# martinhoT/Footsies-Gym

Hardware: NVIDIA B200
Metric: env_frames_per_sec (higher is better)
Workload: dtype int32+fp32

## Files before the change

### footsies_gym_b200/csrc/frame_logic.cuh

```cuda
#ifndef FOOTSIES_B200_FRAME_LOGIC_CUH
#define FOOTSIES_B200_FRAME_LOGIC_CUH

#include <stdint.h>

#include "state_codec.h"

#if defined(__CUDACC__)
#define FG_DEV __device__ __forceinline__
#define FG_ALIGN16 __align__(16)
namespace fg {
FG_DEV float u2f(uint32_t u) { return __uint_as_float(u); }
FG_DEV uint32_t f2u(float f) { return __float_as_uint(f); }
FG_DEV uint32_t umulhi64(uint32_t r, unsigned long long m) { return (uint32_t)__umul64hi((unsigned long long)r, m); }
FG_DEV uint32_t byte_lut(uint32_t lo, uint32_t hi, uint32_t idx) { return __byte_perm(lo, hi, idx); }
FG_DEV uint32_t umin(uint32_t a, uint32_t b) { return min(a, b); }
}
#else
#include <math.h>
#include <string.h>
#define FG_DEV static inline
#define FG_ALIGN16 alignas(16)
struct uint2 { uint32_t x, y; };
struct FG_ALIGN16 uint4 { uint32_t x, y, z, w; };
namespace fg {
FG_DEV float u2f(uint32_t u) { float f; memcpy(&f, &u, 4); return f; }
FG_DEV uint32_t f2u(float f) { uint32_t u; memcpy(&u, &f, 4); return u; }
FG_DEV uint32_t umulhi64(uint32_t r, unsigned long long m) { return (uint32_t)(((unsigned __int128)r * m) >> 64); }
FG_DEV uint32_t byte_lut(uint32_t lo, uint32_t hi, uint32_t idx) {
    const unsigned long long t = (unsigned long long)hi << 32 | lo;
    uint32_t r = 0;
    for (int k = 0; k < 4; k++) r |= (uint32_t)((t >> (8 * ((idx >> (4 * k)) & 7u))) & 0xffu) << (8 * k);
    return r;
}
FG_DEV uint32_t umin(uint32_t a, uint32_t b) { return a < b ? a : b; }
}
#endif

namespace fg {

enum : uint32_t { STAND = FT_IDX_STAND, FORWARD = FT_IDX_FORWARD, BACKWARD = FT_IDX_BACKWARD,
                  DASH_FORWARD = FT_IDX_DASH_FORWARD, DASH_BACKWARD = FT_IDX_DASH_BACKWARD,
                  N_ATTACK = FT_IDX_N_ATTACK, B_ATTACK = FT_IDX_B_ATTACK, N_SPECIAL = FT_IDX_N_SPECIAL,
                  B_SPECIAL = FT_IDX_B_SPECIAL, DAMAGE = FT_IDX_DAMAGE, GUARD_BREAK = FT_IDX_GUARD_BREAK,
                  GUARD_PROXIMITY = FT_IDX_GUARD_PROXIMITY, DEAD = FT_IDX_DEAD, WIN = FT_IDX_WIN };

constexpr int kMovePatBytes = 408;
constexpr int kAttPatBytes = 256;

struct BoxCfg { uint32_t h0cx, h0hw, h1cx, h1hw, pcx, pw, r0, r1; };
struct AttackRow { uint32_t pcx, phw, rcx, rhw, pybits, rybits, result, r0; };
struct BotRow { unsigned long long magic_m, magic_a; uint32_t n_m, sel_m, n_a, sel_a; };

struct FG_ALIGN16 Tables {
    uint4 rows[FT_NUM_ROWS];
    BoxCfg boxcfg[16];
    AttackRow attack[8];
    BotRow bot[8];
    double term_reward[FT_NUM_CUM][4][2];
    double step_reward[4];
    uint8_t cum_next[16][4];
    uint32_t move_meta[8], att_meta[8];
    uint8_t bucket_of[16];
    uint16_t dash_fsm[256][4];
    uint8_t arun_lut[64 * 8];
    uint8_t req_lut[2][1024];
    uint8_t move_pat[2][kMovePatBytes];
    uint8_t att_pat[kAttPatBytes];
};
static_assert(sizeof(Tables) % 16 == 0, "Tables is copied as uint4");
static_assert(sizeof(BoxCfg) == 32 && sizeof(AttackRow) == 32 && sizeof(BotRow) == 32, "byte offsets are pre-positioned");

struct StatAcc { uint32_t a, r, s, ep_frames; };
constexpr uint32_t kStatFlushFrames = 120u;

struct Env {
    float pos1, vel1, pos2, vel2;
    uint32_t pk1, hist1, pk2, hist2;
    int32_t frame;
    uint32_t misc, bq2, bq1;
    uint32_t r0, r1, r2, r3;
    bool drew;
};

constexpr uint32_t M_FRAME1 = 1u << FGP_FRAME_SHIFT, M_ACT = 31u << FGP_ACT_SHIFT, M_STUN = 31u << FGP_STUN_SHIFT,
                   M_STUN1 = 1u << FGP_STUN_SHIFT, M_GUARD = 3u << FGP_GUARD_SHIFT, M_GUARD1 = 1u << FGP_GUARD_SHIFT,
                   M_VITAL = 1u << FGP_VITAL_SHIFT, M_HIT = 1u << FGP_HITCNT_SHIFT, M_BUF = 1u << FGP_BUF_SHIFT,
                   M_RSV = 1u << FGP_RSV_SHIFT, M_INBACK = 1u << FGP_INBACK_SHIFT, M_RPROX = 1u << FGP_RPROX_SHIFT,
                   M_SHMAG = 7u << FGP_SHAKE_SHIFT, M_SHMAG1 = 1u << FGP_SHAKE_SHIFT, M_SHSIGN = 1u << FGP_SHAKE_SIGN_SHIFT;

FG_DEV uint32_t rng_next(Env &e) {
    uint32_t t = e.r0 ^ (e.r0 << 11);
    e.r0 = e.r1; e.r1 = e.r2; e.r2 = e.r3;
    e.r3 = e.r3 ^ (e.r3 >> 19) ^ t ^ (t >> 8);
    e.drew = true;
    return e.r3;
}

struct FrameOut {
    uint32_t z, w;
    float pos_b;
    bool special_started;
    bool from_neutral;
};

template <int SIDE, bool LUT_REQUEST>
FG_DEV void update_fighter(const Tables &T, uint32_t in, float &pos, float &vel, uint32_t &pk, uint32_t &hist, FrameOut &fo) {
    const uint32_t in_lr = in & 3u;
    const uint32_t au = T.arun_lut[((hist >> (FGH_ARUN_SHIFT - 3)) & (63u << 3)) + in];
    const uint32_t du = T.dash_fsm[hist & 255u][in_lr];
    hist = (du & 255u) | (au & 63u) << FGH_ARUN_SHIFT;
    uint32_t delta = (pk & M_STUN) ? (0u - M_STUN1) : M_FRAME1;
    if (pk & M_SHMAG) { delta -= M_SHMAG1; pk ^= M_SHSIGN; }
    pk += delta;
    const bool stun0 = (pk & M_STUN) == 0u;

    uint32_t req;
    bool differs, set, want_buffer;
    if (LUT_REQUEST) {
        static_assert(FGP_RPROX_SHIFT == 23 && FGP_CARRY_END == (1u << 28), "request LUT index assembly");
        const uint32_t ridx = in_lr | ((pk >> 21) & 0x384u) | ((au >> 3) & 0x18u) | ((du >> 3) & 0x60u);
        const uint32_t rq = T.req_lut[SIDE][ridx];
        req = rq & 15u;
        differs = ((pk ^ (req << FGP_ACT_SHIFT)) & M_ACT) != 0u;
        set = (rq & FT_REQ_FREE) && ((rq & FT_REQ_ENDED) || differs);
        want_buffer = (rq & FT_REQ_WANT_BUFFER) != 0u;
    } else {
        const bool special = (au & 64u) != 0u;
        const bool atk_down = (au & 128u) != 0u;
        const bool dash_f = (du & (SIDE == 0 ? 0x200u : 0x100u)) != 0u;
        const bool dash_b = (du & (SIDE == 0 ? 0x100u : 0x200u)) != 0u;
        const bool ended = (pk & FGP_CARRY_END) != 0u;
        const bool in_normal = (pk & FGP_CARRY_NORMAL) && !ended;
        const uint32_t dir = in_lr != 0u ? 1u : 0u;
        const uint32_t areq = special ? N_SPECIAL + dir : in_normal ? (uint32_t)N_SPECIAL : N_ATTACK + dir;
        const uint32_t mv = byte_lut(SIDE == 0 ? 0x00010200u : 0x00020100u, SIDE == 0 ? 0x00010e00u : 0x000e0100u,
                                     in_lr | ((pk >> (FGP_RPROX_SHIFT - 2)) & 4u));
        req = (special || atk_down) ? areq : dash_f ? (uint32_t)DASH_FORWARD : dash_b ? (uint32_t)DASH_BACKWARD : mv;
        const bool free_to_switch = ended || (pk & FGP_CARRY_ALWAYS);
        differs = ((pk ^ (req << FGP_ACT_SHIFT)) & M_ACT) != 0u;
        set = free_to_switch && (ended || differs);
        want_buffer = !free_to_switch && req == N_SPECIAL;
    }
    const bool normal = (pk & FGP_CARRY_NORMAL) != 0u;
    if ((pk & (M_RSV | M_BUF)) && stun0 && ((pk & M_RSV) || (pk & M_HIT))) {
        req = (pk & M_RSV) ? (uint32_t)GUARD_BREAK : (uint32_t)N_SPECIAL;
        set = true; differs = true; want_buffer = false;
    } else {
        pk = (pk & ~(M_INBACK | M_RPROX)) | (in & (SIDE == 0 ? 1u : 2u)) << (FGP_INBACK_SHIFT - (SIDE == 0 ? 0 : 1));
    }
    if (SIDE == 0) {
        fo.special_started = set && differs && (req - N_SPECIAL) < 2u;
        fo.from_neutral = !normal;
    }
    if (set) pk = (pk & (M_STUN | M_GUARD | M_VITAL | M_INBACK | M_RPROX)) + (req << FGP_ACT_SHIFT);

    const uint4 row = T.rows[pk & FGP_ROW_MASK];
    if (want_buffer) pk |= (row.z & FT_Z_CANCEL) << (FGP_BUF_SHIFT - 3);
    pk = (pk & ~FGP_CARRY_MASK) | (row.w & (stun0 ? FGP_CARRY_MASK : (FGP_CARRY_MASK & ~FGP_CARRY_END)));

    if (stun0) {
        const float dx = u2f(row.x);
        pos = pos + (SIDE == 0 ? dx : -dx);
        if (row.z & FT_Z_HAS_MOVEMENT) vel = u2f(row.y);
    }
    fo.z = row.z;
    fo.w = row.w;
    fo.pos_b = pos;
}

FG_DEV const BoxCfg &boxcfg_of(const Tables &T, uint32_t z) {
    return *reinterpret_cast<const BoxCfg *>(reinterpret_cast<const char *>(T.boxcfg) + (z & (15u << FT_Z_BOXCFG_SHIFT)));
}
FG_DEV const AttackRow &attack_of(const Tables &T, uint32_t w) {
    return *reinterpret_cast<const AttackRow *>(reinterpret_cast<const char *>(T.attack) + (w & (7u << FT_W_KIND_SHIFT)));
}
static_assert(FT_Z_BOXCFG_SHIFT == 5 && FT_W_KIND_SHIFT == 5, "id << 5 == byte offset of a 32-byte table row");
static_assert(FT_Z_CANCEL == 8u, "update_fighter shifts the cancel bit into the buffered-cancel bit");

template <int SIDE>
FG_DEV void box_extent(float pos_b, uint32_t cx_bits, uint32_t hw_bits, float s, float t, float &lo, float &hi) {
    const float cx = u2f(cx_bits), hw = u2f(hw_bits);
    const float x = ((pos_b + (SIDE == 0 ? cx : -cx)) + s) + t;
    lo = x - hw;
    hi = x + hw;
}

template <int ASIDE>
FG_DEV void attack_overlaps(const AttackRow &ar, const BoxCfg &vb, const FrameOut &af, const FrameOut &vf, float a_s,
                            float a_t, float v_s, float v_t, bool &real_hit, bool &prox_hit) {
    float plo, phi, rlo, rhi, v0lo, v0hi, v1lo, v1hi;
    box_extent<ASIDE>(af.pos_b, ar.pcx, ar.phw, a_s, a_t, plo, phi);
    box_extent<ASIDE>(af.pos_b, ar.rcx, ar.rhw, a_s, a_t, rlo, rhi);
    box_extent<1 - ASIDE>(vf.pos_b, vb.h0cx, vb.h0hw, v_s, v_t, v0lo, v0hi);
    box_extent<1 - ASIDE>(vf.pos_b, vb.h1cx, vb.h1hw, v_s, v_t, v1lo, v1hi);
    constexpr uint32_t Y0 = 0xffu << FT_Z_YMASK0_SHIFT, Y1 = 0xffu << FT_Z_YMASK1_SHIFT;
    const bool r0 = (vf.z & ar.rybits & Y0) && v0hi >= rlo && v0lo <= rhi;
    const bool r1 = (vf.z & ar.rybits & Y1) && v1hi >= rlo && v1lo <= rhi;
    const bool p0 = (vf.z & ar.pybits & Y0) && v0hi >= plo && v0lo <= phi;
    const bool p1 = (vf.z & ar.pybits & Y1) && v1hi >= plo && v1lo <= phi;
    real_hit = (af.z & FT_Z_REAL) && (r0 || r1);
    prox_hit = (af.z & FT_Z_PROX) && (p0 || p1);
}

template <int ASIDE>
FG_DEV uint32_t attack_apply(uint32_t result, uint32_t &apk, uint32_t &vpk, const FrameOut &af, const FrameOut &vf,
                             bool real_hit, bool prox_hit, StatAcc &acc) {
    const bool can = (af.z & (FT_Z_PROX | FT_Z_REAL)) && !(apk & M_HIT);
    if (can && real_hit) {
        const bool brk = (vpk & M_GUARD) == 0u;
        const bool guarding = (vf.z & FT_Z_GUARDING) != 0u;
        uint32_t nact, stun, res;
        uint32_t keep = vpk & (M_GUARD | M_VITAL | M_INBACK | M_RPROX);
        if (!brk) keep -= M_GUARD1;
        if (guarding) {
            nact = (result >> 5) & 31u;
            stun = brk ? (result >> 21) & 31u : (result >> 16) & 31u;
            if (brk) keep |= M_RSV;
            res = brk ? 3u : 6u;
            acc.r += brk ? (1u << 24) : (1u << 16);
        } else {
            if (result & (1u << 10)) keep &= ~M_VITAL;
            nact = result & 31u;
            stun = (result >> 11) & 31u;
            res = brk ? 1u : 5u;
            acc.r += 1u << 8;
        }
        const uint32_t mag = umin(stun / 3u, 6u);
        vpk = keep | nact << FGP_ACT_SHIFT | stun << FGP_STUN_SHIFT | mag << FGP_SHAKE_SHIFT
            | (ASIDE == 0 ? 0u : (mag ? M_SHSIGN : 0u));
        apk = (apk & ~(M_STUN | (stun ? FGP_CARRY_END : 0u))) | stun << FGP_STUN_SHIFT | M_HIT;
        return res;
    }
    if (can && prox_hit) vpk |= (vpk & M_INBACK) << (FGP_RPROX_SHIFT - FGP_INBACK_SHIFT);
    return 0u;
}

FG_DEV uint32_t bot_dist_index(float dist) {
    float t2 = dist * 2.0f;
    t2 = t2 < 4.0f ? 4.0f : t2 > 9.0f ? 9.0f : t2;
    return (uint32_t)((int)ceilf(t2) - 4);
}
FG_DEV float bot_dist_of_index(uint32_t idx) { return 0.5f * (float)(idx + 4u); }

template <int SIDE>
FG_DEV uint32_t bot_next(const Tables &T, Env &e, uint32_t &q, float dist, uint32_t opp_act) {
    uint32_t input = 0u;
    const bool have_m = (q & (127u << 9)) != 0u, have_a = (q & (127u << 24)) != 0u;
    if (have_m) {
        input = T.move_pat[SIDE][q & 511u];
        q += 1u - (1u << 9);
    }
    if (have_a) {
        input |= T.att_pat[(q >> 16) & 255u];
        q += (1u << 16) - (1u << 24);
    }
    if (!(have_m && have_a)) {
        const BotRow &b = T.bot[T.bucket_of[bot_dist_index(dist)]];
        if (!have_m) {
            const uint32_t r = rng_next(e);
            const uint32_t k = r - umulhi64(r, b.magic_m) * b.n_m;
            const uint32_t meta = T.move_meta[(b.sel_m >> (4u * k)) & 15u];
            q = (q & 0xffff0000u) | (meta & 0xffffu) | (meta >> 16) << 9;
        }
        if (!have_a) {
            const bool opp_hurt = opp_act == DAMAGE || opp_act == GUARD_BREAK || opp_act == N_SPECIAL || opp_act == B_SPECIAL;
            const bool opp_normal = opp_act == N_ATTACK || opp_act == B_ATTACK;
            uint32_t ap = 3u;
            if (!(opp_hurt || (opp_normal && (b.n_a >> 8)))) {
                const uint32_t r = rng_next(e);
                const uint32_t n = b.n_a & 255u;
                const uint32_t k = r - umulhi64(r, b.magic_a) * n;
                ap = (b.sel_a >> (4u * k)) & 15u;
            }
            const uint32_t meta = T.att_meta[ap];
            q = (q & 0x0000ffffu) | (meta & 0xffffu) << 16 | (meta >> 16) << 24;
        }
    }
    return input;
}

template <bool P1BOT, bool P2BOT>
FG_DEV void reset_env(const Tables &T, Env &e, bool stale_intro) {
    const bool was_done = (e.misc >> FGM_DONE_SHIFT) & 1u;
    uint32_t a1 = (e.misc >> FGM_ACTOR1_SHIFT) & 7u, a2 = (e.misc >> FGM_ACTOR2_SHIFT) & 7u;
    if (!stale_intro) { a1 = 0u; a2 = 0u; }
    float p1_dist = 0.0f;
    uint32_t p1_opp = 0u;
    bool p1_called = false;
    if (P1BOT) {
        p1_called = (e.misc >> FGM_P1CALLED_SHIFT) & 1u;
        p1_dist = was_done ? bot_dist_of_index((e.misc >> FGM_P1MEM_SHIFT) & 7u) : fabsf(e.pos2 - e.pos1);
        p1_opp = was_done ? (e.misc >> (FGM_P1MEM_SHIFT + 3)) & 31u : (e.pk2 >> FGP_ACT_SHIFT) & 31u;
    }
    uint32_t pk[2] = { e.pk1, e.pk2 };
    uint32_t npk[2];
#pragma unroll
    for (int s = 0; s < 2; s++) {
        uint32_t stun = (pk[s] >> FGP_STUN_SHIFT) & 31u;
        uint32_t keep = pk[s] & (M_INBACK | M_RPROX);
        if (was_done) {
            if (stun > 0u) stun--;
            if (!(pk[s] & M_VITAL)) keep = 0u;
        }
        uint32_t frame = 1u;
        if (stun > 0u) { stun--; frame = 0u; }
        npk[s] = STAND << FGP_ACT_SHIFT | frame << FGP_FRAME_SHIFT | stun << FGP_STUN_SHIFT | 3u << FGP_GUARD_SHIFT
               | M_VITAL | keep | FGP_CARRY_ALWAYS;
    }
    e.pk1 = npk[0]; e.pk2 = npk[1];
    e.pos1 = -2.0f; e.pos2 = 2.0f; e.vel1 = 0.0f; e.vel2 = 0.0f;
    e.hist1 = (T.dash_fsm[0][a1 & 3u] & 255u) | ((a1 >> 2) & 1u) << FGH_ARUN_SHIFT;
    e.hist2 = (T.dash_fsm[0][a2 & 3u] & 255u) | ((a2 >> 2) & 1u) << FGH_ARUN_SHIFT;
    e.frame = -1;
    e.bq2 = 0u;
    if (!P1BOT) e.bq1 = 0u;
    if (P1BOT) a1 = p1_called ? bot_next<0>(T, e, e.bq1, p1_dist, p1_opp) : 0u;
    if (P2BOT) a2 = bot_next<1>(T, e, e.bq2, 4.0f, STAND);
    e.misc = a1 << FGM_ACTOR1_SHIFT | a2 << FGM_ACTOR2_SHIFT
           | (P1BOT ? 1u << FGM_P1CALLED_SHIFT : 0u);
}

struct StepOutputs {
    float obs[8];
    uint32_t info_misc;
};
FG_DEV void make_outputs(const Env &e, StepOutputs &o) {
    uint32_t m1 = (e.pk1 >> FGP_ACT_SHIFT) & 31u, m2 = (e.pk2 >> FGP_ACT_SHIFT) & 31u;
    if (m1 >= DEAD) m1 = STAND;
    if (m2 >= DEAD) m2 = STAND;
    const uint32_t f1 = m1 <= BACKWARD ? 0u : e.pk1 & 63u;
    const uint32_t f2 = m2 <= BACKWARD ? 0u : e.pk2 & 63u;
    o.obs[0] = (float)((e.pk1 >> FGP_GUARD_SHIFT) & 3u); o.obs[1] = (float)((e.pk2 >> FGP_GUARD_SHIFT) & 3u);
    o.obs[2] = (float)m1; o.obs[3] = (float)m2;
    o.obs[4] = (float)f1; o.obs[5] = (float)f2; o.obs[6] = e.pos1; o.obs[7] = e.pos2;
    o.info_misc = ((e.misc >> FGM_REC1_SHIFT) & 7u) | ((e.misc >> FGM_REC2_SHIFT) & 7u) << 8
                | ((e.pk1 >> FGP_STUN_SHIFT) & 31u) << 16 | ((e.pk2 >> FGP_STUN_SHIFT) & 31u) << 24;
}

FG_DEV bool obs_is_skippable(const Env &e) {
    uint32_t m1 = (e.pk1 >> FGP_ACT_SHIFT) & 31u, m2 = (e.pk2 >> FGP_ACT_SHIFT) & 31u;
    if (m1 >= DEAD) m1 = STAND;
    if (m2 >= DEAD) m2 = STAND;
    const uint32_t f1 = m1 <= BACKWARD ? 0u : e.pk1 & 63u;
    const bool p2_hit_guard = m2 == DAMAGE || m2 == FT_IDX_GUARD_STAND || m2 == FT_IDX_GUARD_CROUCH || m2 == FT_IDX_GUARD_M || m2 == GUARD_BREAK;
    return (f1 != 0u && !p2_hit_guard) || m1 == DAMAGE;
}

template <bool P1BOT, bool P2BOT, bool DENSE, bool LUT_REQUEST>
FG_DEV void simulate_frame(const Tables &T, Env &e, uint32_t in1, uint32_t in2, double &reward, bool &terminal, StatAcc &acc) {
    float pre_dist = 0.0f;
    uint32_t pre_a1 = 0u, pre_a2 = 0u;
    if (P1BOT || P2BOT) {
        pre_dist = fabsf(e.pos2 - e.pos1);
        pre_a1 = (e.pk1 >> FGP_ACT_SHIFT) & 31u;
        pre_a2 = (e.pk2 >> FGP_ACT_SHIFT) & 31u;
    }

    e.frame++;
    if (e.frame < FG_MAX_RECORDING_INPUT_FRAME)
        e.misc = (e.misc & ~(63u << FGM_REC1_SHIFT)) | (in1 + in2 * 8u) << FGM_REC1_SHIFT;

    FrameOut f1, f2;
    update_fighter<0, LUT_REQUEST>(T, in1, e.pos1, e.vel1, e.pk1, e.hist1, f1);
    update_fighter<1, LUT_REQUEST>(T, in2, e.pos2, e.vel2, e.pk2, e.hist2, f2);

    const BoxCfg &b1 = boxcfg_of(T, f1.z), &b2 = boxcfg_of(T, f2.z);
    const float px1 = e.pos1 + u2f(b1.pcx), w1 = u2f(b1.pw);
    const float px2 = e.pos2 - u2f(b2.pcx), w2 = u2f(b2.pw);
    const float xmax1 = w1 + px1, xmax2 = w2 + px2;
    float s1 = 0.0f, s2 = 0.0f;
    if (xmax2 > px1 && px2 < xmax1) {
        if (e.pos1 < e.pos2) { const float d = xmax1 - px2; s1 = -0.5f * d; s2 = 0.5f * d; }
        else if (e.pos1 > e.pos2) { const float d = xmax2 - px1; s1 = 0.5f * d; s2 = -0.5f * d; }
    }
    float t1 = 0.0f, t2 = 0.0f;
    {
        const float c = px1 + s1, hw = 0.5f * w1, mn = c - hw, mx = c + hw;
        if (mn < -5.0f) t1 = -5.0f - mn; else if (mx > 5.0f) t1 = 5.0f - mx;
    }
    {
        const float c = px2 + s2, hw = 0.5f * w2, mn = c - hw, mx = c + hw;
        if (mn < -5.0f) t2 = -5.0f - mn; else if (mx > 5.0f) t2 = 5.0f - mx;
    }
    e.pos1 = (e.pos1 + s1) + t1;
    e.pos2 = (e.pos2 + s2) + t2;

    uint32_t res_a = 0u, res_b = 0u;
    if ((f1.z | f2.z) & (FT_Z_PROX | FT_Z_REAL)) {
        const AttackRow &ar1 = attack_of(T, f1.w), &ar2 = attack_of(T, f2.w);
        bool real_a, prox_a, real_b, prox_b;
        attack_overlaps<0>(ar1, b2, f1, f2, s1, t1, s2, t2, real_a, prox_a);
        attack_overlaps<1>(ar2, b1, f2, f1, s2, t2, s1, t1, real_b, prox_b);
        res_a = attack_apply<0>(ar1.result, e.pk1, e.pk2, f1, f2, real_a, prox_a, acc);
        res_b = attack_apply<1>(ar2.result, e.pk2, e.pk1, f2, f1, real_b, prox_b, acc);
    }

    if (f1.special_started && res_b == 0u) acc.s += f1.from_neutral ? 0x101u : 1u;

    terminal = ((e.pk1 & e.pk2) & M_VITAL) == 0u;

    if (DENSE) {
        const uint32_t code = (res_b >> 2) | (res_a >> 2) << 1;
        if (code | (terminal ? 1u : 0u)) {
            const uint32_t cum = T.cum_next[(e.misc >> FGM_CUM_SHIFT) & 15u][code];
            e.misc = (e.misc & ~(15u << FGM_CUM_SHIFT)) | cum << FGM_CUM_SHIFT;
            reward += terminal ? T.term_reward[cum][code][(e.pk2 & M_VITAL) ? 0 : 1] : T.step_reward[code];
        }
    } else if (terminal) {
        reward += (e.pk2 & M_VITAL) ? -1.0 : 1.0;
    }

    uint32_t n1 = in1, n2 = in2;
    if (terminal) {
        const bool dead1 = !(e.pk1 & M_VITAL), dead2 = !(e.pk2 & M_VITAL);
        e.hist1 = 0u; e.hist2 = 0u;
        acc.a += 1u + (1u << (8u * (dead1 && dead2 ? 3u : dead2 ? 1u : 2u)));
        acc.ep_frames += (uint32_t)(e.frame + 1);
        e.misc |= 1u << FGM_DONE_SHIFT;
        if (P1BOT) e.misc = (e.misc & ~(255u << FGM_P1MEM_SHIFT)) | (bot_dist_index(pre_dist) | pre_a2 << 3) << FGM_P1MEM_SHIFT;
    } else {
        if (P1BOT) n1 = bot_next<0>(T, e, e.bq1, pre_dist, pre_a2);
        if (P2BOT) n2 = bot_next<1>(T, e, e.bq2, pre_dist, pre_a1);
    }
    e.misc = (e.misc & ~(63u << FGM_ACTOR1_SHIFT)) | (n1 + n2 * 8u) << FGM_ACTOR1_SHIFT;
}

}
#endif
```

### footsies_gym_b200/csrc/step_kernel.cuh

```cuda
#ifndef FOOTSIES_B200_STEP_KERNEL_CUH
#define FOOTSIES_B200_STEP_KERNEL_CUH
#include "device_once.h"
#include <cuda_runtime.h>
#include <stdint.h>
#include <stdio.h>
#include <string.h>
#include <new>
#include <vector>

#include "tables_host.h"

namespace fgk {

using namespace fg;

template <int THREADS_, int GROUP_, int STAGES_, int MIN_BLOCKS_>
struct StepShape {
    static constexpr int kThreads = THREADS_, kGroupThreads = GROUP_, kGroups = THREADS_ / GROUP_, kStages = STAGES_,
                         kMinBlocks = MIN_BLOCKS_;
    static_assert(THREADS_ % GROUP_ == 0 && GROUP_ % 32 == 0, "groups are whole warps");
};
#if defined(FG_THREADS)
#ifndef FG_GROUP
#define FG_GROUP FG_THREADS
#endif
#ifndef FG_STAGES
#define FG_STAGES 2
#endif
#ifndef FG_BLOCKS_PER_SM
#define FG_BLOCKS_PER_SM 4
#endif
using ShapeSmall = StepShape<FG_THREADS, FG_GROUP, FG_STAGES, FG_BLOCKS_PER_SM>;
using ShapeLargeSingle = ShapeSmall;
using ShapeLargeFused = ShapeSmall;
#else
using ShapeSmall = StepShape<256, 256, 2, 3>;
using ShapeLargeSingle = StepShape<768, 256, 3, 1>;
using ShapeLargeFused = StepShape<1024, 256, 3, 1>;
#endif
constexpr int kLargeShapeMinEnvs = 768 * 1024;
#ifndef FG_SKIP_RNG_STORE
#define FG_SKIP_RNG_STORE 1
#endif
#ifndef FG_PDL
#define FG_PDL 1
#endif
#ifndef FG_REVERSE
#define FG_REVERSE 1
#endif
constexpr int kThreads = 256;
constexpr uint32_t kFull = 0xffffffffu;

struct Params {
    uint4 *pl_f1, *pl_f2, *pl_env, *pl_rng;
    unsigned long long *stats;
    const uint8_t *act1, *act2;
    float4 *obs;
    float *reward;
    uint8_t *terminated;
    int32_t *info_frame;
    uint32_t *info_misc;
    const Tables *tables;
    const uint8_t *mask;
    const uint8_t *step_mask;
    long long seed_base, first_env_index;
    int n, frame_skip, autoreset, stale_intro;
    int skip_unactionable;
    int large_shape_min_envs;
    int reverse;
    int pdl;
    int pdl_min_envs;
};

__device__ __forceinline__ void write_outputs(const Params &p, int i, const Env &e, float reward, bool terminated) {
    StepOutputs o;
    make_outputs(e, o);
    p.obs[2 * (size_t)i] = make_float4(o.obs[0], o.obs[1], o.obs[2], o.obs[3]);
    p.obs[2 * (size_t)i + 1] = make_float4(o.obs[4], o.obs[5], o.obs[6], o.obs[7]);
    p.reward[i] = reward;
    p.terminated[i] = terminated ? 1 : 0;
    p.info_frame[i] = e.frame;
    p.info_misc[i] = o.info_misc;
}

__device__ __forceinline__ void load_tables(Tables *dst, const Tables *src) {
    const uint4 *s = reinterpret_cast<const uint4 *>(src);
    uint4 *d = reinterpret_cast<uint4 *>(dst);
    for (int k = threadIdx.x; k < (int)(sizeof(Tables) / 16); k += blockDim.x) d[k] = s[k];
}

template <bool WITH_RNG>
__device__ __forceinline__ void load_env(const Params &p, int i, Env &e) {
    const uint4 a = p.pl_f1[i], b = p.pl_f2[i], c = p.pl_env[i];
    e.pos1 = u2f(a.x); e.vel1 = u2f(a.y); e.pk1 = a.z; e.hist1 = a.w;
    e.pos2 = u2f(b.x); e.vel2 = u2f(b.y); e.pk2 = b.z; e.hist2 = b.w;
    e.frame = (int32_t)c.x; e.misc = c.y; e.bq2 = c.z; e.bq1 = c.w;
    if (WITH_RNG) { const uint4 r = p.pl_rng[i]; e.r0 = r.x; e.r1 = r.y; e.r2 = r.z; e.r3 = r.w; }
    e.drew = false;
}
template <bool WITH_RNG>
__device__ __forceinline__ void store_env(const Params &p, int i, const Env &e) {
    p.pl_f1[i] = make_uint4(f2u(e.pos1), f2u(e.vel1), e.pk1, e.hist1);
    p.pl_f2[i] = make_uint4(f2u(e.pos2), f2u(e.vel2), e.pk2, e.hist2);
    p.pl_env[i] = make_uint4((uint32_t)e.frame, e.misc, e.bq2, e.bq1);
    if (WITH_RNG && (!FG_SKIP_RNG_STORE || e.drew)) p.pl_rng[i] = make_uint4(e.r0, e.r1, e.r2, e.r3);
}

__device__ __forceinline__ void flush_stats(StatAcc &acc, unsigned long long *s_stats, int lane) {
    const uint32_t w[3] = { acc.a, acc.r, acc.s };
    const int map[3][4] = { { FG_STAT_EPISODES, FG_STAT_P1_WINS, FG_STAT_P2_WINS, FG_STAT_DOUBLE_KO },
                            { -1, FG_STAT_HITS, FG_STAT_BLOCKS, FG_STAT_GUARD_BREAKS },
                                            { FG_STAT_P1_SPECIALS, FG_STAT_P1_SPECIALS_NEUTRAL, FG_STAT_RESETS, FG_STAT_ENV_FRAMES } };
#pragma unroll
    for (int k = 0; k < 3; k++)
#pragma unroll
        for (int b = 0; b < 4; b++) {
            if (map[k][b] < 0) continue;
            const uint32_t tot = __reduce_add_sync(kFull, (w[k] >> (8 * b)) & 255u);
            if (lane == 0 && tot) atomicAdd(&s_stats[map[k][b]], (unsigned long long)tot);
        }
    const uint32_t lo = __reduce_add_sync(kFull, acc.ep_frames & 0xffffu), hi = __reduce_add_sync(kFull, acc.ep_frames >> 16);
    if (lane == 0 && (lo | hi)) atomicAdd(&s_stats[FG_STAT_EPISODE_FRAMES], ((unsigned long long)hi << 16) + lo);
    acc.a = 0u; acc.r = 0u; acc.s = 0u; acc.ep_frames = 0u;
}

__device__ __forceinline__ uint32_t smem_u32(const void *p) { return (uint32_t)__cvta_generic_to_shared(p); }
__device__ __forceinline__ void mbar_init(uint64_t *bar, uint32_t count) {
    asm volatile("mbarrier.init.shared::cta.b64 [%0], %1;" ::"r"(smem_u32(bar)), "r"(count));
}
__device__ __forceinline__ void mbar_expect_tx(uint64_t *bar, uint32_t bytes) {
    asm volatile("mbarrier.arrive.expect_tx.shared::cta.b64 _, [%0], %1;" ::"r"(smem_u32(bar)), "r"(bytes) : "memory");
}
__device__ __forceinline__ void mbar_arrive(uint64_t *bar) {
    asm volatile("mbarrier.arrive.shared::cta.b64 _, [%0];" ::"r"(smem_u32(bar)) : "memory");
}
__device__ __forceinline__ void mbar_wait(uint64_t *bar, uint32_t parity) {
    asm volatile(
        "{\n"
        ".reg .pred P1;\n"
        "LAB_WAIT:\n"
        "mbarrier.try_wait.parity.shared::cta.b64 P1, [%0], %1;\n"
        "@P1 bra DONE;\n"
        "bra LAB_WAIT;\n"
        "DONE:\n"
        "}" ::"r"(smem_u32(bar)), "r"(parity) : "memory");
}
__device__ __forceinline__ void tma_load_1d(void *dst, const void *src, uint32_t bytes, uint64_t *bar) {
    asm volatile("cp.async.bulk.shared::cluster.global.mbarrier::complete_tx::bytes [%0], [%1], %2, [%3];"
                 ::"r"(smem_u32(dst)), "l"(src), "r"(bytes), "r"(smem_u32(bar)) : "memory");
}

template <class SH, int PLANES>
struct __align__(128) StepSmem {
    Tables T;
    uint4 stage[SH::kGroups][SH::kStages][PLANES][SH::kGroupThreads];
    uint64_t full_bar[SH::kGroups][SH::kStages], empty_bar[SH::kGroups][SH::kStages];
    unsigned long long stats[FG_STAT_COUNT];
};

template <class SH, bool KFUSED, bool P1BOT, bool P2BOT, bool DENSE, bool MASKED>
__global__ void __launch_bounds__(SH::kThreads, SH::kMinBlocks) step_kernel(const Params p) {
    constexpr bool kRng = P1BOT || P2BOT;
    constexpr int kPlanes = kRng ? 4 : 3;
    constexpr int kGroupThreads = SH::kGroupThreads, kGroups = SH::kGroups, kStages = SH::kStages;
    extern __shared__ __align__(128) unsigned char smem_raw[];
    StepSmem<SH, kPlanes> &S = *reinterpret_cast<StepSmem<SH, kPlanes> *>(smem_raw);
    const Tables &T = S.T;
    const int lane = threadIdx.x & 31;
    const int g = threadIdx.x / kGroupThreads, lt = threadIdx.x % kGroupThreads;
    const int num_chunks = (p.n + kGroupThreads - 1) / kGroupThreads;
    const int full_chunks = p.n / kGroupThreads;
    const int first = blockIdx.x * kGroups + g, stride = gridDim.x * kGroups;
    const uint4 *const planes[4] = { p.pl_f1, p.pl_f2, p.pl_env, p.pl_rng };
    auto issue = [&](int chunk, int s) {
        mbar_expect_tx(&S.full_bar[g][s], (uint32_t)(kPlanes * kGroupThreads * sizeof(uint4)));
#pragma unroll
        for (int k = 0; k < kPlanes; k++)
            tma_load_1d(S.stage[g][s][k], planes[k] + (size_t)chunk * kGroupThreads, (uint32_t)(kGroupThreads * sizeof(uint4)),
                        &S.full_bar[g][s]);
    };
    auto chunk_of = [&](int c) { return (FG_REVERSE && p.reverse && c < full_chunks) ? full_chunks - 1 - c : c; };
    if (lt == 0) {
        for (int s = 0; s < kStages; s++) { mbar_init(&S.full_bar[g][s], 1u); mbar_init(&S.empty_bar[g][s], kGroupThreads / 32); }
        asm volatile("fence.mbarrier_init.release.cluster;" ::: "memory");
    }
    if (FG_PDL && p.pdl) {
        load_tables(&S.T, p.tables);
        if (threadIdx.x < FG_STAT_COUNT) S.stats[threadIdx.x] = 0ull;
        asm volatile("griddepcontrol.launch_dependents;" ::: "memory");
        asm volatile("griddepcontrol.wait;" ::: "memory");
    }
    if (lt == 0) {
        for (int j = 0; j < kStages - 1; j++) {
            const int cj = first + j * stride;
            if (cj < num_chunks && chunk_of(cj) < full_chunks) issue(chunk_of(cj), j);
        }
    }
    if (!(FG_PDL && p.pdl)) {
        load_tables(&S.T, p.tables);
        if (threadIdx.x < FG_STAT_COUNT) S.stats[threadIdx.x] = 0ull;
    }
    __syncthreads();
    StatAcc acc = { 0u, 0u, 0u, 0u };
    uint32_t frames_since_flush = 0u;
    uint32_t nin1 = 0u, nin2 = 0u;
    {
        const int i0 = (first < num_chunks ? chunk_of(first) : num_chunks) * kGroupThreads + lt;
        if (i0 < p.n) { if (!P1BOT) nin1 = p.act1[i0]; if (!P2BOT) nin2 = p.act2[i0]; }
    }
    int k = 0;
    for (int cl = first; cl < num_chunks; cl += stride, k++) {
        const int s = k % kStages;
        const int c = chunk_of(cl);
        const int i = c * kGroupThreads + lt;
        const bool staged = c < full_chunks;
        bool valid = staged || i < p.n;
        if (MASKED) valid = valid && p.step_mask[valid ? i : 0] != 0;
        if (lt == 0) {
            const int cn = cl + (kStages - 1) * stride;
            if (cn < num_chunks && chunk_of(cn) < full_chunks) {
                const int sn = (k + kStages - 1) % kStages;
                if (k >= 1) mbar_wait(&S.empty_bar[g][sn], ((k - 1) / kStages) & 1);
                issue(chunk_of(cn), sn);
            }
        }
        const uint32_t act1 = nin1, act2 = nin2;
        {
            const int cn1 = cl + stride;
            const int in = (cn1 < num_chunks ? chunk_of(cn1) : num_chunks) * kGroupThreads + lt;
            if (in < p.n) { if (!P1BOT) nin1 = p.act1[in]; if (!P2BOT) nin2 = p.act2[in]; }
        }
        Env e;
        bool run = false;
        uint32_t in1 = 0u, in2 = 0u;
        if (staged) {
            mbar_wait(&S.full_bar[g][s], (k / kStages) & 1);
            const uint4 a = S.stage[g][s][0][lt], b = S.stage[g][s][1][lt], cc = S.stage[g][s][2][lt];
            e.pos1 = u2f(a.x); e.vel1 = u2f(a.y); e.pk1 = a.z; e.hist1 = a.w;
            e.pos2 = u2f(b.x); e.vel2 = u2f(b.y); e.pk2 = b.z; e.hist2 = b.w;
            e.frame = (int32_t)cc.x; e.misc = cc.y; e.bq2 = cc.z; e.bq1 = cc.w;
            if (kRng) { const uint4 r = S.stage[g][s][kPlanes - 1][lt]; e.r0 = r.x; e.r1 = r.y; e.r2 = r.z; e.r3 = r.w; }
            e.drew = false;
            __syncwarp();
            if (lane == 0) mbar_arrive(&S.empty_bar[g][s]);
        } else if (valid) {
            load_env<kRng>(p, i, e);
        }
        if (valid) {
            if ((e.misc >> FGM_DONE_SHIFT) & 1u) {
                if (p.autoreset) {
                    reset_env<P1BOT, P2BOT>(T, e, p.stale_intro != 0);
                    store_env<kRng>(p, i, e);
                    write_outputs(p, i, e, 0.0f, false);
                    acc.s += 0x10000u;
                } else {
                    p.reward[i] = 0.0f;
                }
            } else {
                run = true;
                in1 = P1BOT ? (e.misc >> FGM_ACTOR1_SHIFT) & 7u : act1 & 7u;
                in2 = P2BOT ? (e.misc >> FGM_ACTOR2_SHIFT) & 7u : act2 & 7u;
            }
        }
        double reward = 0.0;
        bool terminal = false;
        const int K = KFUSED ? p.frame_skip : 1;
        for (int kk = 0; kk < K; kk++) {
            if (run && !terminal) {
                simulate_frame<P1BOT, P2BOT, DENSE, KFUSED>(T, e, in1, in2, reward, terminal, acc);
                acc.s += 1u << 24;
                if (KFUSED) {
                    if (P1BOT) in1 = (e.misc >> FGM_ACTOR1_SHIFT) & 7u;
                    if (P2BOT) in2 = (e.misc >> FGM_ACTOR2_SHIFT) & 7u;
                }
            }
        }
        if (KFUSED && p.skip_unactionable) {
            bool more = run && !terminal && obs_is_skippable(e);
            while (__any_sync(kFull, more)) {
                for (int kk = 0; kk < K; kk++) {
                    if (more && !terminal) {
                        simulate_frame<P1BOT, P2BOT, DENSE, KFUSED>(T, e, 0u, in2, reward, terminal, acc);
                        acc.s += 1u << 24;
                        if (P2BOT) in2 = (e.misc >> FGM_ACTOR2_SHIFT) & 7u;
                    }
                }
                more = more && !terminal && obs_is_skippable(e);
                frames_since_flush += (uint32_t)K;
                if (frames_since_flush >= kStatFlushFrames) { flush_stats(acc, S.stats, lane); frames_since_flush = 0u; }
            }
        }
        if (run) {
            store_env<kRng>(p, i, e);
            write_outputs(p, i, e, (float)reward, terminal);
        }
        frames_since_flush += (uint32_t)K;
        if (frames_since_flush >= kStatFlushFrames) { flush_stats(acc, S.stats, lane); frames_since_flush = 0u; }
    }
    flush_stats(acc, S.stats, lane);
    __syncthreads();
    if (threadIdx.x < FG_STAT_COUNT && S.stats[threadIdx.x]) atomicAdd(&p.stats[threadIdx.x], S.stats[threadIdx.x]);
}

template <bool P1BOT, bool P2BOT>
__global__ void __launch_bounds__(kThreads) reset_kernel(const Params p) {
    extern __shared__ __align__(128) unsigned char smem_raw[];
    Tables &T = *reinterpret_cast<Tables *>(smem_raw);
    load_tables(&T, p.tables);
    __syncthreads();
    constexpr bool kRng = P1BOT || P2BOT;
    unsigned long long resets = 0ull;
    for (int i = blockIdx.x * blockDim.x + threadIdx.x; i < p.n; i += gridDim.x * blockDim.x) {
        if (p.mask && !p.mask[i]) continue;
        Env e;
        load_env<kRng>(p, i, e);
        reset_env<P1BOT, P2BOT>(T, e, p.stale_intro != 0);
        store_env<kRng>(p, i, e);
        write_outputs(p, i, e, 0.0f, false);
        resets++;
    }
    if (resets) atomicAdd(&p.stats[FG_STAT_RESETS], resets);
}

static __global__ void __launch_bounds__(kThreads) seed_kernel(const Params p) {
    for (int i = blockIdx.x * blockDim.x + threadIdx.x; i < p.n; i += gridDim.x * blockDim.x) {
        if (p.mask && !p.mask[i]) continue;
        uint32_t s0 = (uint32_t)(int32_t)(p.seed_base + p.first_env_index + i);
        uint32_t s1 = s0 * 1812433253u + 1u, s2 = s1 * 1812433253u + 1u, s3 = s2 * 1812433253u + 1u;
        p.pl_rng[i] = make_uint4(s0, s1, s2, s3);
    }
}

template <class SH, bool KF, bool B1, bool B2, bool D, bool M>
cudaError_t launch_step_shape(int sm_count, cudaStream_t s, const Params &p) {
    constexpr int kPlanes = (B1 || B2) ? 4 : 3;
    constexpr size_t bytes = sizeof(StepSmem<SH, kPlanes>);
    static DeviceOnceFlags configured;
    if (cudaError_t e = configure_once_per_device(configured, [] {
            return cudaFuncSetAttribute(step_kernel<SH, KF, B1, B2, D, M>, cudaFuncAttributeMaxDynamicSharedMemorySize, (int)bytes); }))
        return e;
    const int want = (p.n + SH::kThreads - 1) / SH::kThreads, cap = sm_count * SH::kMinBlocks;
    const int grid = want < cap ? (want > 0 ? want : 1) : cap;
#if FG_PDL
    if (!p.pdl) {
        step_kernel<SH, KF, B1, B2, D, M><<<grid, SH::kThreads, bytes, s>>>(p);
        return cudaSuccess;
    }
    cudaLaunchConfig_t cfg = {};
    cfg.gridDim = dim3((unsigned)grid);
    cfg.blockDim = dim3((unsigned)SH::kThreads);
    cfg.dynamicSmemBytes = bytes;
    cfg.stream = s;
    cudaLaunchAttribute attr[1];
    attr[0].id = cudaLaunchAttributeProgrammaticStreamSerialization;
    attr[0].val.programmaticStreamSerializationAllowed = 1;
    cfg.attrs = attr;
    cfg.numAttrs = 1;
    return cudaLaunchKernelEx(&cfg, step_kernel<SH, KF, B1, B2, D, M>, p);
#else
    step_kernel<SH, KF, B1, B2, D, M><<<grid, SH::kThreads, bytes, s>>>(p);
    return cudaSuccess;
#endif
}
template <bool KF, bool B1, bool B2, bool D, bool M>
cudaError_t launch_step(int sm_count, cudaStream_t s, const Params &p) {
    if (p.n < p.large_shape_min_envs) return launch_step_shape<ShapeSmall, KF, B1, B2, D, M>(sm_count, s, p);
    if (KF) return launch_step_shape<ShapeLargeFused, KF, B1, B2, D, M>(sm_count, s, p);
    return launch_step_shape<ShapeLargeSingle, KF, B1, B2, D, M>(sm_count, s, p);
}
template <bool KF, bool B1, bool B2>
cudaError_t launch_step_d(bool dense, bool masked, int sm_count, cudaStream_t s, const Params &p) {
    if (dense) return masked ? launch_step<KF, B1, B2, true, true>(sm_count, s, p) : launch_step<KF, B1, B2, true, false>(sm_count, s, p);
    return masked ? launch_step<KF, B1, B2, false, true>(sm_count, s, p) : launch_step<KF, B1, B2, false, false>(sm_count, s, p);
}
#ifndef FG_STEP_INSTANCE
extern template cudaError_t launch_step_d<false, false, false>(bool, bool, int, cudaStream_t, const Params &);
extern template cudaError_t launch_step_d<false, false, true>(bool, bool, int, cudaStream_t, const Params &);
extern template cudaError_t launch_step_d<false, true, false>(bool, bool, int, cudaStream_t, const Params &);
extern template cudaError_t launch_step_d<false, true, true>(bool, bool, int, cudaStream_t, const Params &);
extern template cudaError_t launch_step_d<true, false, false>(bool, bool, int, cudaStream_t, const Params &);
extern template cudaError_t launch_step_d<true, false, true>(bool, bool, int, cudaStream_t, const Params &);
extern template cudaError_t launch_step_d<true, true, false>(bool, bool, int, cudaStream_t, const Params &);
extern template cudaError_t launch_step_d<true, true, true>(bool, bool, int, cudaStream_t, const Params &);
#endif

}
#endif
```

Before: 34.31 billion.

## Fetch per-env RNG state on demand only when a bot may draw

Removes the RNG plane from the bulk TMA stream in the non-fused bot kernels. Each lane instead issues a predicated cp.async that reads its RNG state only when the env is done or a bot action queue is empty, and zero-fills otherwise. The fetch is double-buffered one chunk ahead. This cuts global read bandwidth for envs that will not draw random numbers, at the cost of an extra wait on the next stage's barrier, per-lane async copies, and extra shared memory.

```diff
diff --git a/footsies_gym_b200/csrc/frame_logic.cuh b/footsies_gym_b200/csrc/frame_logic.cuh
--- a/footsies_gym_b200/csrc/frame_logic.cuh
+++ b/footsies_gym_b200/csrc/frame_logic.cuh
@@ -280,6 +280,12 @@
 }
 
 template <bool P1BOT, bool P2BOT>
+FG_DEV bool step_may_draw(uint32_t misc, uint32_t bq1, uint32_t bq2) {
+    const auto empty = [](uint32_t q) { return (q & (127u << 9)) == 0u || (q & (127u << 24)) == 0u; };
+    return ((misc >> FGM_DONE_SHIFT) & 1u) || (P1BOT && empty(bq1)) || (P2BOT && empty(bq2));
+}
+
+template <bool P1BOT, bool P2BOT>
 FG_DEV void reset_env(const Tables &T, Env &e, bool stale_intro) {
     const bool was_done = (e.misc >> FGM_DONE_SHIFT) & 1u;
     uint32_t a1 = (e.misc >> FGM_ACTOR1_SHIFT) & 7u, a2 = (e.misc >> FGM_ACTOR2_SHIFT) & 7u;
diff --git a/footsies_gym_b200/csrc/step_kernel.cuh b/footsies_gym_b200/csrc/step_kernel.cuh
--- a/footsies_gym_b200/csrc/step_kernel.cuh
+++ b/footsies_gym_b200/csrc/step_kernel.cuh
@@ -47,6 +47,12 @@
 #endif
 #ifndef FG_REVERSE
 #define FG_REVERSE 1
+#endif
+#ifndef FG_RNG_ON_DEMAND
+#define FG_RNG_ON_DEMAND 1
+#endif
+#if FG_RNG_ON_DEMAND && !FG_SKIP_RNG_STORE
+#error "FG_RNG_ON_DEMAND needs FG_SKIP_RNG_STORE: a lane that did not fetch its RNG state must not write it back"
 #endif
 constexpr int kThreads = 256;
 constexpr uint32_t kFull = 0xffffffffu;
@@ -149,6 +155,18 @@
     asm volatile("cp.async.bulk.shared::cluster.global.mbarrier::complete_tx::bytes [%0], [%1], %2, [%3];"
                  ::"r"(smem_u32(dst)), "l"(src), "r"(bytes), "r"(smem_u32(bar)) : "memory");
 }
+__device__ __forceinline__ void cp_async_16_or_zero(void *dst, const void *src, bool fetch) {
+    asm volatile("cp.async.cg.shared.global [%0], [%1], 16, %2;" ::"r"(smem_u32(dst)), "l"(src), "r"(fetch ? 16 : 0) : "memory");
+}
+__device__ __forceinline__ void cp_async_commit() { asm volatile("cp.async.commit_group;" ::: "memory"); }
+__device__ __forceinline__ void cp_async_wait_prev() { asm volatile("cp.async.wait_group 1;" ::: "memory"); }
+
+template <class SH, bool KFUSED, bool P1BOT, bool P2BOT>
+struct StepPlanes {
+    static constexpr bool kRng = P1BOT || P2BOT, kRngOnDemand = FG_RNG_ON_DEMAND && !KFUSED && kRng;
+    static constexpr int kStreamed = kRng && !kRngOnDemand ? 4 : 3;
+    static constexpr size_t kRngSlotBytes = kRngOnDemand ? (size_t)SH::kGroups * 2 * SH::kGroupThreads * sizeof(uint4) : 0;
+};
 
 template <class SH, int PLANES>
 struct __align__(128) StepSmem {
@@ -160,14 +178,16 @@
 
 template <class SH, bool KFUSED, bool P1BOT, bool P2BOT, bool DENSE, bool MASKED>
 __global__ void __launch_bounds__(SH::kThreads, SH::kMinBlocks) step_kernel(const Params p) {
-    constexpr bool kRng = P1BOT || P2BOT;
-    constexpr int kPlanes = kRng ? 4 : 3;
+    using PL = StepPlanes<SH, KFUSED, P1BOT, P2BOT>;
+    constexpr bool kRng = PL::kRng, kRngOnDemand = PL::kRngOnDemand;
+    constexpr int kPlanes = PL::kStreamed;
     constexpr int kGroupThreads = SH::kGroupThreads, kGroups = SH::kGroups, kStages = SH::kStages;
     extern __shared__ __align__(128) unsigned char smem_raw[];
     StepSmem<SH, kPlanes> &S = *reinterpret_cast<StepSmem<SH, kPlanes> *>(smem_raw);
     const Tables &T = S.T;
     const int lane = threadIdx.x & 31;
     const int g = threadIdx.x / kGroupThreads, lt = threadIdx.x % kGroupThreads;
+    uint4 *const rng_slot = reinterpret_cast<uint4 *>(smem_raw + sizeof(StepSmem<SH, kPlanes>)) + (size_t)g * 2 * kGroupThreads;
     const int num_chunks = (p.n + kGroupThreads - 1) / kGroupThreads;
     const int full_chunks = p.n / kGroupThreads;
     const int first = blockIdx.x * kGroups + g, stride = gridDim.x * kGroups;
@@ -180,6 +200,13 @@
                         &S.full_bar[g][s]);
     };
     auto chunk_of = [&](int c) { return (FG_REVERSE && p.reverse && c < full_chunks) ? full_chunks - 1 - c : c; };
+    auto fetch_rng = [&](int cl_, int kk) {
+        const int s_ = kk % kStages;
+        mbar_wait(&S.full_bar[g][s_], (kk / kStages) & 1);
+        const uint4 w = S.stage[g][s_][2][lt];
+        cp_async_16_or_zero(&rng_slot[(kk & 1) * kGroupThreads + lt], p.pl_rng + (size_t)chunk_of(cl_) * kGroupThreads + lt,
+                            step_may_draw<P1BOT, P2BOT>(w.y, w.w, w.z));
+    };
     if (lt == 0) {
         for (int s = 0; s < kStages; s++) { mbar_init(&S.full_bar[g][s], 1u); mbar_init(&S.empty_bar[g][s], kGroupThreads / 32); }
         asm volatile("fence.mbarrier_init.release.cluster;" ::: "memory");
@@ -239,7 +266,17 @@
             e.pos1 = u2f(a.x); e.vel1 = u2f(a.y); e.pk1 = a.z; e.hist1 = a.w;
             e.pos2 = u2f(b.x); e.vel2 = u2f(b.y); e.pk2 = b.z; e.hist2 = b.w;
             e.frame = (int32_t)cc.x; e.misc = cc.y; e.bq2 = cc.z; e.bq1 = cc.w;
-            if (kRng) { const uint4 r = S.stage[g][s][kPlanes - 1][lt]; e.r0 = r.x; e.r1 = r.y; e.r2 = r.z; e.r3 = r.w; }
+            if (kRngOnDemand) {
+                if (k == 0) { fetch_rng(cl, 0); cp_async_commit(); }
+                const int cn1 = cl + stride;
+                if (cn1 < num_chunks && chunk_of(cn1) < full_chunks) fetch_rng(cn1, k + 1);
+                cp_async_commit();
+                cp_async_wait_prev();
+                const uint4 r = rng_slot[(k & 1) * kGroupThreads + lt];
+                e.r0 = r.x; e.r1 = r.y; e.r2 = r.z; e.r3 = r.w;
+            } else if (kRng) {
+                const uint4 r = S.stage[g][s][kPlanes - 1][lt]; e.r0 = r.x; e.r1 = r.y; e.r2 = r.z; e.r3 = r.w;
+            }
             e.drew = false;
             __syncwarp();
             if (lane == 0) mbar_arrive(&S.empty_bar[g][s]);
@@ -333,8 +370,8 @@
 
 template <class SH, bool KF, bool B1, bool B2, bool D, bool M>
 cudaError_t launch_step_shape(int sm_count, cudaStream_t s, const Params &p) {
-    constexpr int kPlanes = (B1 || B2) ? 4 : 3;
-    constexpr size_t bytes = sizeof(StepSmem<SH, kPlanes>);
+    using PL = StepPlanes<SH, KF, B1, B2>;
+    constexpr size_t bytes = sizeof(StepSmem<SH, PL::kStreamed>) + PL::kRngSlotBytes;
     static DeviceOnceFlags configured;
     if (cudaError_t e = configure_once_per_device(configured, [] {
             return cudaFuncSetAttribute(step_kernel<SH, KF, B1, B2, D, M>, cudaFuncAttributeMaxDynamicSharedMemorySize, (int)bytes); }))
```

Result: slower. 32.97 billion (median of 6 runs) (-3.9%).
